# aalobaidi/ggRMCP

Hardware: AMD Instinct MI355X
Metric: MCP tool_call→gRPC unary req/sec (whole node) (higher is better)
Workload: dtype uint8; 1 GPU; model=hello-service SayHello (HTTP serving), global_batch=1024, seq_len=1024, parallelism=dp1, mode=serving-gpu, sessions=1024, payload_bytes=1024, backend=local grpc over uds, separate process (native) x1, transport=native, http=native frontend, C++ closed-loop client

## Files before the change

### ggrmcp_amd/backend/native_invoker.py

```python

from __future__ import annotations

import logging
from typing import Dict, List, Optional, Sequence, Tuple

log = logging.getLogger("ggrmcp.native_invoker")

_CODE_NAMES = [
    "OK", "CANCELLED", "UNKNOWN", "INVALID_ARGUMENT", "DEADLINE_EXCEEDED",
    "NOT_FOUND", "ALREADY_EXISTS", "PERMISSION_DENIED", "RESOURCE_EXHAUSTED",
    "FAILED_PRECONDITION", "ABORTED", "OUT_OF_RANGE", "UNIMPLEMENTED",
    "INTERNAL", "UNAVAILABLE", "DATA_LOSS", "UNAUTHENTICATED",
]


class _Code:
    def __init__(self, value: int) -> None:
        self.value = value
        self.name = (
            _CODE_NAMES[value] if 0 <= value < len(_CODE_NAMES) else f"CODE_{value}"
        )


class NativeRpcError(Exception):

    def __init__(self, code: int, message: str) -> None:
        super().__init__(f"{_Code(code).name}: {message}")
        self._code = _Code(code)
        self._message = message

    def code(self) -> _Code:
        return self._code

    def details(self) -> str:
        return self._message


def load_module():
    import importlib
    import sys
    from pathlib import Path

    ops_dir = str(Path(__file__).resolve().parent.parent / "ops")
    if ops_dir not in sys.path:
        sys.path.insert(0, ops_dir)
    return importlib.import_module("_h2grpc")


class NativeWireClient:

    def __init__(self, target: str, connections: int = 8, authority: str = "",
                 max_inflight: int = 512, max_resp_bytes: int = 0) -> None:
        mod = load_module()
        self.target = target
        self._cli = mod.Client(target, connections=connections,
                               authority=authority or "localhost",
                               max_inflight=max_inflight,
                               max_resp_bytes=max_resp_bytes)

    def invoke_batch(
        self,
        paths: Sequence[str],
        payloads: Sequence[bytes],
        timeout_s: float,
        metadata: Optional[Sequence[Sequence[Tuple[str, str]]]] = None,
    ) -> List[object]:
        res = self._cli.invoke_batch(
            list(paths), list(payloads), timeout_s, list(metadata or [])
        )
        out: List[object] = []
        for status, payload, message in res:
            if status == 0:
                out.append(payload)
            else:
                out.append(NativeRpcError(status, message))
        return out

    def invoke_stream_batch(
        self,
        paths: Sequence[str],
        payloads: Sequence[bytes],
        timeout_s: float,
        metadata: Optional[Sequence[Sequence[Tuple[str, str]]]] = None,
    ) -> List[object]:
        res = self._cli.invoke_stream_batch(
            list(paths), list(payloads), timeout_s, list(metadata or [])
        )
        out: List[object] = []
        for status, blob, lens, message in res:
            if status == 0:
                mv = memoryview(blob)
                chunks = []
                off = 0
                for ln in lens:
                    chunks.append(mv[off : off + ln])
                    off += ln
                out.append(chunks)
            else:
                out.append(NativeRpcError(status, message))
        return out

    def healthy(self) -> bool:
        return self._cli.healthy()

    def close(self) -> None:
        self._cli.close()
```

### ggrmcp_amd/ops/csrc/h2grpc.cpp

```cpp

#include "h2grpc_impl.h"

PYBIND11_MODULE(_h2grpc, m) {
  m.doc() = "native gRPC-over-HTTP/2 transport (nghttp2): batch client + bench server";
  py::class_<H2GrpcClient>(m, "Client")
      .def(py::init<const std::string&, int, const std::string&, int, size_t>(),
           py::arg("target"), py::arg("connections") = 4, py::arg("authority") = "",
           py::arg("max_inflight") = 512, py::arg("max_resp_bytes") = 0)
      .def("invoke_stream_batch", &H2GrpcClient::invoke_stream_batch,
           py::arg("paths"), py::arg("payloads"), py::arg("timeout_s") = 30.0,
           py::arg("metadata") = std::vector<std::vector<std::pair<std::string, std::string>>>{})
      .def("invoke_batch", &H2GrpcClient::invoke_batch, py::arg("paths"),
           py::arg("payloads"), py::arg("timeout_s") = 30.0,
           py::arg("metadata") = std::vector<std::vector<std::pair<std::string, std::string>>>{})
      .def("healthy", &H2GrpcClient::healthy)
      .def("raw_handle",
           [](H2GrpcClient& c) { return (uintptr_t)&c; },
           "opaque H2GrpcClient* for the native span executor; the client "
           "must outlive every frontend/engine holding the handle")
      .def("close", &H2GrpcClient::close_all);
  py::class_<H2Server>(m, "Server")
      .def(py::init<const std::string&>(), py::arg("target"))
      .def("add_route", &H2Server::add_route, py::arg("path"), py::arg("kind"))
      .def("request_count", &H2Server::request_count)
      .def("start", &H2Server::start)
      .def("stop", &H2Server::stop);
}
```

### ggrmcp_amd/ops/csrc/h2grpc_impl.h

```cpp
#pragma once

#include <arpa/inet.h>
#include <errno.h>
#include <fcntl.h>
#include <netinet/in.h>
#include <netinet/tcp.h>
#include <nghttp2/nghttp2.h>
#include <poll.h>
#include <pybind11/pybind11.h>
#include <pybind11/stl.h>
#include <string.h>
#include <stdio.h>
#include <stdlib.h>
#include <sys/eventfd.h>
#include <sys/socket.h>
#include <sys/un.h>
#include <unistd.h>

#include <atomic>
#include <chrono>
#include <condition_variable>
#include <cstdint>
#include <deque>
#include <memory>
#include <mutex>
#include <stdexcept>
#include <string>
#include <thread>
#include <unordered_map>
#include <vector>

namespace py = pybind11;
using Clock = std::chrono::steady_clock;


static int transport_sockbuf() {
  const char* e = getenv("GGRMCP_SOCKBUF");
  return e ? atoi(e) : (4 << 20);
}

static void apply_sockbuf(int fd) {
  int sz = transport_sockbuf();
  if (sz > 0) {
    setsockopt(fd, SOL_SOCKET, SO_SNDBUF, &sz, sizeof(sz));
    setsockopt(fd, SOL_SOCKET, SO_RCVBUF, &sz, sizeof(sz));
  }
}

static int connect_target(const std::string& target) {
  int fd = -1;
  if (target.rfind("unix:", 0) == 0) {
    fd = socket(AF_UNIX, SOCK_STREAM, 0);
    if (fd < 0) throw std::runtime_error("socket() failed");
    sockaddr_un addr{};
    addr.sun_family = AF_UNIX;
    std::string path = target.substr(5);
    if (path.size() >= sizeof(addr.sun_path)) throw std::runtime_error("uds path too long");
    memcpy(addr.sun_path, path.c_str(), path.size() + 1);
    apply_sockbuf(fd);
    if (connect(fd, (sockaddr*)&addr, sizeof(addr)) != 0) {
      close(fd);
      throw std::runtime_error("connect failed: " + target);
    }
  } else {
    auto colon = target.rfind(':');
    if (colon == std::string::npos) throw std::runtime_error("bad target " + target);
    std::string host = target.substr(0, colon);
    int port = std::stoi(target.substr(colon + 1));
    fd = socket(AF_INET, SOCK_STREAM, 0);
    if (fd < 0) throw std::runtime_error("socket() failed");
    sockaddr_in addr{};
    addr.sin_family = AF_INET;
    addr.sin_port = htons((uint16_t)port);
    if (inet_pton(AF_INET, host.c_str(), &addr.sin_addr) != 1) {
      close(fd);
      throw std::runtime_error("bad host (use a literal IP): " + host);
    }
    apply_sockbuf(fd);
    if (connect(fd, (sockaddr*)&addr, sizeof(addr)) != 0) {
      close(fd);
      throw std::runtime_error("connect failed: " + target);
    }
    int one = 1;
    setsockopt(fd, IPPROTO_TCP, TCP_NODELAY, &one, sizeof(one));
  }
  int flags = fcntl(fd, F_GETFL, 0);
  fcntl(fd, F_SETFL, flags | O_NONBLOCK);
  return fd;
}

#define NV(NAME, VALUE, NLEN, VLEN)                                      \
  nghttp2_nv {                                                           \
    (uint8_t*)(NAME), (uint8_t*)(VALUE), (size_t)(NLEN), (size_t)(VLEN), \
        NGHTTP2_NV_FLAG_NONE                                             \
  }

static nghttp2_nv nv(const char* name, const char* value) {
  return NV(name, value, strlen(name), strlen(value));
}
static nghttp2_nv nv(const char* name, const std::string& value) {
  return NV(name, value.data(), strlen(name), value.size());
}
static nghttp2_nv nv(const std::string& name, const std::string& value) {
  return NV(name.data(), value.data(), name.size(), value.size());
}

static std::string grpc_frame(const std::string& payload) {
  std::string out;
  out.resize(5 + payload.size());
  out[0] = 0;
  uint32_t n = htonl((uint32_t)payload.size());
  memcpy(&out[1], &n, 4);
  memcpy(&out[5], payload.data(), payload.size());
  return out;
}

static bool pb_validate(const uint8_t* p, size_t len) {
  size_t pos = 0;
  int depth_guard = 0;
  while (pos < len) {
    uint64_t tag = 0;
    int shift = 0;
    bool done = false;
    while (pos < len && shift <= 63) {
      uint8_t b = p[pos++];
      tag |= (uint64_t)(b & 0x7F) << shift;
      if (!(b & 0x80)) { done = true; break; }
      shift += 7;
    }
    if (!done) return false;
    uint32_t wt = tag & 7;
    if ((tag >> 3) == 0) return false;
    switch (wt) {
      case 0: {
        bool vdone = false;
        for (int i = 0; i < 10 && pos < len; ++i) {
          if (!(p[pos++] & 0x80)) { vdone = true; break; }
        }
        if (!vdone) return false;
        break;
      }
      case 1: if (pos + 8 > len) return false; pos += 8; break;
      case 5: if (pos + 4 > len) return false; pos += 4; break;
      case 2: {
        uint64_t l = 0;
        int s2 = 0;
        bool d2 = false;
        while (pos < len && s2 <= 35) {
          uint8_t b = p[pos++];
          l |= (uint64_t)(b & 0x7F) << s2;
          if (!(b & 0x80)) { d2 = true; break; }
          s2 += 7;
        }
        if (!d2 || pos + l > len) return false;
        pos += l;
        break;
      }
      default: return false;
    }
    if (++depth_guard > 1'000'000) return false;
  }
  return true;
}

static bool parse_hello_name(const uint8_t* p, size_t len, std::string* name) {
  size_t pos = 0;
  while (pos < len) {
    uint64_t tag = 0;
    int shift = 0;
    bool done = false;
    while (pos < len && shift <= 63) {
      uint8_t b = p[pos++];
      tag |= (uint64_t)(b & 0x7F) << shift;
      if (!(b & 0x80)) { done = true; break; }
      shift += 7;
    }
    if (!done) return false;
    if ((tag >> 3) == 1 && (tag & 7) == 2) {
      uint64_t l = 0;
      int s2 = 0;
      bool d2 = false;
      while (pos < len && s2 <= 35) {
        uint8_t b = p[pos++];
        l |= (uint64_t)(b & 0x7F) << s2;
        if (!(b & 0x80)) { d2 = true; break; }
        s2 += 7;
      }
      if (!d2 || pos + l > len) return false;
      name->assign((const char*)p + pos, l);
      pos += l;
    } else {
      uint32_t wt = tag & 7;
      if (wt == 0) {
        while (pos < len && (p[pos++] & 0x80)) {}
      } else if (wt == 1) {
        pos += 8;
      } else if (wt == 5) {
        pos += 4;
      } else if (wt == 2) {
        uint64_t l = 0;
        int s2 = 0;
        while (pos < len && s2 <= 35) {
          uint8_t b = p[pos++];
          l |= (uint64_t)(b & 0x7F) << s2;
          if (!(b & 0x80)) break;
          s2 += 7;
        }
        pos += l;
      } else {
        return false;
      }
    }
  }
  return true;
}

static std::string make_hello_response(const std::string& name) {
  std::string msg = "Hello, " + name + "!";
  std::string out;
  out.push_back('\x0a');
  uint64_t v = msg.size();
  while (v >= 0x80) {
    out.push_back((char)(v | 0x80));
    v >>= 7;
  }
  out.push_back((char)v);
  out += msg;
  return out;
}


struct Call {
  std::string path;
  std::string payload;
  size_t sent = 0;
  std::string response;
  int grpc_status = -1;
  std::string grpc_message;
  std::atomic<bool> done{false};
  Clock::time_point deadline;
  int slot = -1;
  bool no_cap = false;
  bool overflow = false;
  std::vector<std::pair<std::string, std::string>> metadata;
};

struct Batch {
  std::deque<Call> calls;
  std::mutex mu;
  std::condition_variable cv;
  std::atomic<int> done{0};
  void complete_one() {
    { std::lock_guard<std::mutex> lk(mu); done.fetch_add(1); }
    cv.notify_one();
  }
};

struct QueuedCall {
  std::shared_ptr<Batch> batch;
  Call* call;
};

struct ClientConn {
  int fd = -1;
  int wake_fd = -1;
  nghttp2_session* sess = nullptr;
  std::thread thread;
  std::mutex mu;
  std::deque<QueuedCall> pending;
  std::unordered_map<int32_t, QueuedCall> live;
  std::string wbuf;
  std::atomic<bool> stop{false};
  std::atomic<int> inflight{0};
  int max_inflight = 512;
  size_t max_resp = 0;
  std::string authority;
  bool broken = false;
};

static ssize_t client_data_read(nghttp2_session*, int32_t stream_id, uint8_t* buf,
                                size_t length, uint32_t* data_flags,
                                nghttp2_data_source* source, void*) {
  Call* call = (Call*)source->ptr;
  size_t left = call->payload.size() - call->sent;
  size_t n = left < length ? left : length;
  memcpy(buf, call->payload.data() + call->sent, n);
  call->sent += n;
  if (call->sent == call->payload.size()) *data_flags |= NGHTTP2_DATA_FLAG_EOF;
  return (ssize_t)n;
}

static int client_on_header(nghttp2_session* sess, const nghttp2_frame* frame,
                            const uint8_t* name, size_t namelen, const uint8_t* value,
                            size_t valuelen, uint8_t, void* user) {
  ClientConn* conn = (ClientConn*)user;
  auto it = conn->live.find(frame->hd.stream_id);
  if (it == conn->live.end()) return 0;
  if (namelen == 11 && memcmp(name, "grpc-status", 11) == 0) {
    it->second.call->grpc_status =
        atoi(std::string((const char*)value, valuelen).c_str());
  } else if (namelen == 12 && memcmp(name, "grpc-message", 12) == 0) {
    it->second.call->grpc_message.assign((const char*)value, valuelen);
  }
  return 0;
}

static int client_on_data(nghttp2_session*, uint8_t, int32_t stream_id,
                          const uint8_t* data, size_t len, void* user) {
  ClientConn* conn = (ClientConn*)user;
  auto it = conn->live.find(stream_id);
  if (it != conn->live.end()) {
    Call* c = it->second.call;
    if (!c->no_cap && conn->max_resp &&
        c->response.size() + len > conn->max_resp) {
      c->overflow = true;
      c->response.clear();
    } else if (!c->overflow) {
      c->response.append((const char*)data, len);
    }
  }
  return 0;
}

static int client_on_stream_close(nghttp2_session*, int32_t stream_id, uint32_t,
                                  void* user) {
  ClientConn* conn = (ClientConn*)user;
  auto it = conn->live.find(stream_id);
  if (it != conn->live.end()) {
    QueuedCall qc = it->second;
    conn->live.erase(it);
    qc.call->done.store(true, std::memory_order_release);
    conn->inflight.fetch_sub(1);
    qc.batch->complete_one();
  }
  return 0;
}

static void fail_call(ClientConn* conn, QueuedCall& qc, int status,
                      const char* msg) {
  qc.call->grpc_status = status;
  qc.call->grpc_message = msg;
  qc.call->done.store(true, std::memory_order_release);
  qc.batch->complete_one();
}


static bool flush_session(nghttp2_session* sess, int fd, std::string& wbuf,
                          bool* blocked) {
  *blocked = false;
  while (true) {
    if (!wbuf.empty()) {
      ssize_t w = send(fd, wbuf.data(), wbuf.size(), MSG_NOSIGNAL);
      if (w < 0) {
        if (errno == EAGAIN || errno == EWOULDBLOCK) { *blocked = true; return true; }
        return false;
      }
      wbuf.erase(0, (size_t)w);
      if (!wbuf.empty()) continue;
    }
    const uint8_t* out = nullptr;
    ssize_t n = nghttp2_session_mem_send(sess, &out);
    if (n < 0) return false;
    if (n == 0) return true;
    ssize_t w = send(fd, out, (size_t)n, MSG_NOSIGNAL);
    if (w < 0) {
      if (errno == EAGAIN || errno == EWOULDBLOCK) w = 0;
      else return false;
    }
    if (w < n) wbuf.assign((const char*)out + w, (size_t)(n - w));
  }
}

static void conn_loop(ClientConn* conn) {
  while (!conn->stop.load()) {
    {
      std::lock_guard<std::mutex> lk(conn->mu);
      while (!conn->pending.empty() &&
             conn->inflight.load() < conn->max_inflight) {
        QueuedCall qc = conn->pending.front();
        Call* call = qc.call;
        conn->pending.pop_front();
        std::vector<nghttp2_nv> nva;
        nva.reserve(8 + call->metadata.size());
        nva.push_back(nv(":method", "POST"));
        nva.push_back(nv(":scheme", "http"));
        nva.push_back(nv(":path", call->path));
        nva.push_back(nv(":authority", conn->authority));
        nva.push_back(nv("te", "trailers"));
        nva.push_back(nv("content-type", "application/grpc"));
        for (auto& kv : call->metadata) nva.push_back(nv(kv.first, kv.second));
        nghttp2_data_provider prd;
        prd.source.ptr = call;
        prd.read_callback = client_data_read;
        int32_t sid = nghttp2_submit_request(conn->sess, nullptr, nva.data(),
                                             nva.size(), &prd, call);
        if (sid < 0) {
          fail_call(conn, qc, 14, "submit failed");
          continue;
        }
        conn->live[sid] = qc;
        conn->inflight.fetch_add(1);
      }
    }
    {
      auto now = Clock::now();
      for (auto& kv : conn->live) {
        if (kv.second.call->deadline < now && kv.second.call->grpc_status < 0) {
          kv.second.call->grpc_status = 4;
          kv.second.call->grpc_message = "deadline exceeded";
          nghttp2_submit_rst_stream(conn->sess, NGHTTP2_FLAG_NONE, kv.first,
                                    NGHTTP2_CANCEL);
        }
      }
    }
    bool write_blocked = false;
    if (!flush_session(conn->sess, conn->fd, conn->wbuf, &write_blocked))
      conn->broken = true;
    if (conn->broken) break;

    pollfd fds[2];
    fds[0] = {conn->fd, (short)(POLLIN | (write_blocked ? POLLOUT : 0)), 0};
    fds[1] = {conn->wake_fd, POLLIN, 0};
    int rc = poll(fds, 2, 100);
    if (rc < 0) break;
    if (fds[1].revents & POLLIN) {
      uint64_t junk;
      while (read(conn->wake_fd, &junk, 8) > 0) {}
    }
    if (fds[0].revents & (POLLIN | POLLERR | POLLHUP)) {
      uint8_t buf[1 << 16];
      while (true) {
        ssize_t r = recv(conn->fd, buf, sizeof(buf), 0);
        if (r > 0) {
          ssize_t consumed = nghttp2_session_mem_recv(conn->sess, buf, r);
          if (consumed < 0) { conn->broken = true; break; }
          if (r < (ssize_t)sizeof(buf)) break;
        } else if (r == 0) {
          conn->broken = true;
          break;
        } else {
          if (errno == EAGAIN || errno == EWOULDBLOCK) break;
          conn->broken = true;
          break;
        }
      }
    }
    if (conn->broken) break;
  }
  std::lock_guard<std::mutex> lk(conn->mu);
  for (auto& kv : conn->live) fail_call(conn, kv.second, 14, "connection lost");
  for (auto& qc : conn->pending) fail_call(conn, qc, 14, "connection lost");
  conn->live.clear();
  conn->pending.clear();
}

class __attribute__((visibility("default"))) H2GrpcClient {
 public:
  H2GrpcClient(const std::string& target, int n_connections,
               const std::string& authority, int max_inflight = 512,
               size_t max_resp_bytes = 0)
      : target_(target) {
    if (n_connections < 1) n_connections = 1;
    for (int i = 0; i < n_connections; ++i) {
      auto conn = std::make_unique<ClientConn>();
      conn->max_inflight = max_inflight < 1 ? 1 : max_inflight;
      conn->max_resp = max_resp_bytes;
      conn->fd = connect_target(target);
      conn->wake_fd = eventfd(0, EFD_NONBLOCK);
      conn->authority = authority.empty() ? "localhost" : authority;

      nghttp2_session_callbacks* cbs;
      nghttp2_session_callbacks_new(&cbs);
      nghttp2_session_callbacks_set_on_header_callback(cbs, client_on_header);
      nghttp2_session_callbacks_set_on_data_chunk_recv_callback(cbs, client_on_data);
      nghttp2_session_callbacks_set_on_stream_close_callback(cbs, client_on_stream_close);
      nghttp2_session_client_new(&conn->sess, cbs, conn.get());
      nghttp2_session_callbacks_del(cbs);

      nghttp2_settings_entry iv[] = {
          {NGHTTP2_SETTINGS_INITIAL_WINDOW_SIZE, (1u << 30)},
          {NGHTTP2_SETTINGS_MAX_CONCURRENT_STREAMS, 8192},
          {NGHTTP2_SETTINGS_MAX_FRAME_SIZE, 1u << 20},
      };
      nghttp2_submit_settings(conn->sess, NGHTTP2_FLAG_NONE, iv, 3);
      nghttp2_session_set_local_window_size(conn->sess, NGHTTP2_FLAG_NONE, 0, 1 << 30);

      ClientConn* raw = conn.get();
      conn->thread = std::thread([raw] { conn_loop(raw); });
      conns_.push_back(std::move(conn));
    }
  }

  ~H2GrpcClient() { close_all(); }

  void close_all() {
    for (auto& conn : conns_) {
      conn->stop.store(true);
      uint64_t one = 1;
      (void)!write(conn->wake_fd, &one, 8);
      if (conn->thread.joinable()) conn->thread.join();
      if (conn->sess) nghttp2_session_del(conn->sess);
      if (conn->fd >= 0) close(conn->fd);
      if (conn->wake_fd >= 0) close(conn->wake_fd);
      conn->sess = nullptr;
      conn->fd = conn->wake_fd = -1;
    }
    conns_.clear();
  }

  bool healthy() const {
    for (auto& conn : conns_)
      if (!conn->broken) return true;
    return false;
  }

// ... 15 lines not shown
      size_t pos = 0;
      bool compressed = false;
      while (pos + 5 <= data.size()) {
        if (data[pos] != 0) {
          compressed = true;
          break;
        }
        uint32_t len;
        memcpy(&len, data.data() + pos + 1, 4);
        len = ntohl(len);
        if (pos + 5 + len > data.size()) break;
        blob.append(data, pos + 5, len);
        lens.push_back(len);
        pos += 5 + len;
      }
      if (status == 0 && compressed) {
        status = 13;
        std::get<2>(r) = "compressed gRPC response frame not supported";
      }
      if (status < 0) {
        status = 2;
        if (std::get<2>(r).empty())
          std::get<2>(r) = "stream closed without grpc-status";
      }
      out.emplace_back(status, py::bytes(blob), std::move(lens), std::get<2>(r));
    }
    return out;
  }

  std::vector<std::tuple<int, py::bytes, std::string>> invoke_batch(
      const std::vector<std::string>& paths, const std::vector<py::bytes>& payloads,
      double timeout_s,
      const std::vector<std::vector<std::pair<std::string, std::string>>>& metadata) {
    auto raw = invoke_collect(paths, payloads, timeout_s, metadata);
    std::vector<std::tuple<int, py::bytes, std::string>> out;
    out.reserve(raw.size());
    for (auto& r : raw) {
      int status = std::get<0>(r);
      const std::string& data = std::get<1>(r);
      std::string payload;
      bool compressed = false;
      if (data.size() >= 5) {
        compressed = data[0] != 0;
        uint32_t len;
        memcpy(&len, data.data() + 1, 4);
        len = ntohl(len);
        if (data.size() >= 5 + (size_t)len) payload = data.substr(5, len);
      }
      if (status < 0) {
        status = 2;
        if (std::get<2>(r).empty())
          std::get<2>(r) = "stream closed without grpc-status";
      } else if (status == 0 && compressed) {
        status = 13;
        std::get<2>(r) = "compressed gRPC response frame not supported";
        payload.clear();
      }
      out.emplace_back(status, py::bytes(payload), std::get<2>(r));
    }
    return out;
  }

 public:
  struct RawCall {
    const char* path;
    size_t path_len;
    const uint8_t* payload;
    size_t payload_len;
    const std::vector<std::pair<std::string, std::string>>* metadata;
  };
  std::vector<std::tuple<int, std::string, std::string>> invoke_raw(
      const std::vector<RawCall>& rc, double timeout_s) {
    size_t n = rc.size();
    auto batch = std::make_shared<Batch>();
    auto deadline = Clock::now() + std::chrono::duration_cast<Clock::duration>(
                                       std::chrono::duration<double>(timeout_s));
    for (size_t i = 0; i < n; ++i) {
      batch->calls.emplace_back();
      Call& call = batch->calls.back();
      call.path.assign(rc[i].path, rc[i].path_len);
      call.deadline = deadline;
      call.slot = (int)i;
      if (rc[i].metadata) call.metadata = *rc[i].metadata;
      call.payload = grpc_frame(
          std::string((const char*)rc[i].payload, rc[i].payload_len));
    }
    size_t nc = conns_.size();
    for (size_t i = 0; i < n; ++i) {
      ClientConn* conn = conns_[i % nc].get();
      std::lock_guard<std::mutex> lk(conn->mu);
      conn->pending.push_back(QueuedCall{batch, &batch->calls[i]});
    }
    for (auto& conn : conns_) {
      uint64_t one = 1;
      (void)!write(conn->wake_fd, &one, 8);
    }
    {
      std::unique_lock<std::mutex> lk(batch->mu);
      auto hard = deadline + std::chrono::seconds(2);
      while (batch->done.load() < (int)n) {
        if (batch->cv.wait_until(lk, hard) == std::cv_status::timeout) break;
      }
    }
    std::vector<std::tuple<int, std::string, std::string>> out;
    out.reserve(n);
    for (size_t i = 0; i < n; ++i) {
      Call& call = batch->calls[i];
      if (!call.done.load(std::memory_order_acquire)) {
        out.emplace_back(4, std::string(), "deadline exceeded");
        continue;
      }
      if (call.overflow) {
        out.emplace_back(8, std::string(),
                         "response exceeds max_recv_msg_bytes");
        continue;
      }
      out.emplace_back(call.grpc_status, std::move(call.response),
                       call.grpc_message);
    }
    return out;
  }

 private:
  std::vector<std::tuple<int, std::string, std::string>> invoke_collect(
      const std::vector<std::string>& paths, const std::vector<py::bytes>& payloads,
      double timeout_s,
      const std::vector<std::vector<std::pair<std::string, std::string>>>& metadata,
      bool no_cap = false) {
    size_t n = paths.size();
    if (payloads.size() != n) throw std::runtime_error("paths/payloads mismatch");
    auto batch = std::make_shared<Batch>();
    auto deadline = Clock::now() + std::chrono::duration_cast<Clock::duration>(
                                       std::chrono::duration<double>(timeout_s));
    for (size_t i = 0; i < n; ++i) {
      batch->calls.emplace_back();
      Call& call = batch->calls.back();
      call.path = paths[i];
      call.deadline = deadline;
      call.slot = (int)i;
      call.no_cap = no_cap;
      if (i < metadata.size()) call.metadata = metadata[i];
      std::string raw = payloads[i];
      call.payload = grpc_frame(raw);
    }
    {
      py::gil_scoped_release rel;
      size_t nc = conns_.size();
      for (size_t i = 0; i < n; ++i) {
        ClientConn* conn = conns_[i % nc].get();
        std::lock_guard<std::mutex> lk(conn->mu);
        conn->pending.push_back(QueuedCall{batch, &batch->calls[i]});
      }
      for (auto& conn : conns_) {
        uint64_t one = 1;
        (void)!write(conn->wake_fd, &one, 8);
      }
      std::unique_lock<std::mutex> lk(batch->mu);
      auto hard = deadline + std::chrono::seconds(2);
      while (batch->done.load() < (int)n) {
        if (batch->cv.wait_until(lk, hard) == std::cv_status::timeout) break;
      }
    }
    std::vector<std::tuple<int, std::string, std::string>> out;
    out.reserve(n);
    for (size_t i = 0; i < n; ++i) {
      Call& call = batch->calls[i];
      if (!call.done.load(std::memory_order_acquire)) {
        out.emplace_back(4, std::string(), "deadline exceeded");
        continue;
      }
      if (call.overflow) {
        out.emplace_back(8, std::string(),
                         "response exceeds max_recv_msg_bytes");
        continue;
      }
      out.emplace_back(call.grpc_status, std::move(call.response),
                       call.grpc_message);
    }
    return out;
  }

 public:

 private:
  std::string target_;
  std::vector<std::unique_ptr<ClientConn>> conns_;
};


struct ServerStream {
  std::string path;
  std::string body;
  std::string response;
  size_t sent = 0;
  int grpc_status = 0;
  std::string grpc_message;
  bool responded = false;
};

struct ServerConn {
  int fd = -1;
  nghttp2_session* sess = nullptr;
  std::unordered_map<int32_t, ServerStream> streams;
  std::string wbuf;
  bool broken = false;
  class H2Server* server = nullptr;
};

class H2Server {
 public:
  std::unordered_map<std::string, int> routes;

  H2Server(const std::string& target) : target_(target) {}

  ~H2Server() { stop(); }

  void add_route(const std::string& path, const std::string& kind) {
    routes[path] = (kind == "hello") ? 1 : (kind == "stream_echo") ? 2 : 0;
  }

  std::string start() {
    if (target_.rfind("unix:", 0) == 0) {
      listen_fd_ = socket(AF_UNIX, SOCK_STREAM, 0);
      sockaddr_un addr{};
      addr.sun_family = AF_UNIX;
      std::string path = target_.substr(5);
      if (path.size() >= sizeof(addr.sun_path))
        throw std::runtime_error("uds path too long: " + path);
      unlink(path.c_str());
      memcpy(addr.sun_path, path.c_str(), path.size() + 1);
      if (bind(listen_fd_, (sockaddr*)&addr, sizeof(addr)) != 0)
        throw std::runtime_error("bind failed: " + target_);
      bound_ = target_;
    } else {
      auto colon = target_.rfind(':');
      std::string host = target_.substr(0, colon);
      int port = std::stoi(target_.substr(colon + 1));
      listen_fd_ = socket(AF_INET, SOCK_STREAM, 0);
      int one = 1;
      setsockopt(listen_fd_, SOL_SOCKET, SO_REUSEADDR, &one, sizeof(one));
      sockaddr_in addr{};
      addr.sin_family = AF_INET;
      addr.sin_port = htons((uint16_t)port);
      inet_pton(AF_INET, host.c_str(), &addr.sin_addr);
      if (bind(listen_fd_, (sockaddr*)&addr, sizeof(addr)) != 0)
        throw std::runtime_error("bind failed: " + target_);
      socklen_t alen = sizeof(addr);
      getsockname(listen_fd_, (sockaddr*)&addr, &alen);
      bound_ = host + ":" + std::to_string(ntohs(addr.sin_port));
    }
    if (listen(listen_fd_, 512) != 0) throw std::runtime_error("listen failed");
    int flags = fcntl(listen_fd_, F_GETFL, 0);
    fcntl(listen_fd_, F_SETFL, flags | O_NONBLOCK);
    stop_.store(false);
    accept_thread_ = std::thread([this] { accept_loop(); });
    return bound_;
  }

  void stop() {
    if (stop_.exchange(true)) return;
    if (accept_thread_.joinable()) accept_thread_.join();
    if (listen_fd_ >= 0) close(listen_fd_);
    listen_fd_ = -1;
  }

  long request_count() const { return requests_.load(); }

  void handle(ServerStream& st) {
    requests_.fetch_add(1, std::memory_order_relaxed);
    auto it = routes.find(st.path);
    if (it == routes.end()) {
      st.grpc_status = 12;
      st.grpc_message = "unknown method " + st.path;
      return;
    }
    if (st.body.size() < 5) {
      st.grpc_status = 13;
      st.grpc_message = "truncated grpc frame";
      return;
    }
    uint32_t len;
    memcpy(&len, st.body.data() + 1, 4);
    len = ntohl(len);
    if (st.body.size() < 5 + (size_t)len) {
      st.grpc_status = 13;
      st.grpc_message = "short grpc frame";
      return;
    }
    const uint8_t* msg = (const uint8_t*)st.body.data() + 5;
    if (it->second == 2) {
      if (!pb_validate(msg, len)) {
        st.grpc_status = 13;
        st.grpc_message = "malformed protobuf";
        return;
      }
      int64_t count = 1;
      {
        size_t pos = 0;
        while (pos < len) {
          uint64_t tag = 0;
          int shift = 0;
          while (pos < len && shift <= 63) {
            uint8_t b = msg[pos++];
            tag |= (uint64_t)(b & 0x7F) << shift;
            if (!(b & 0x80)) break;
            shift += 7;
          }
          uint32_t num = (uint32_t)(tag >> 3), wt = (uint32_t)(tag & 7);
          if (num == 2 && wt == 0) {
            uint64_t v = 0;
            int s2 = 0;
            while (pos < len && s2 <= 63) {
              uint8_t b = msg[pos++];
              v |= (uint64_t)(b & 0x7F) << s2;
              if (!(b & 0x80)) break;
              s2 += 7;
            }
            count = (int64_t)(int32_t)(uint32_t)v;
            break;
          }
          if (wt == 0) {
            while (pos < len && (msg[pos++] & 0x80)) {}
          } else if (wt == 1) {
            pos += 8;
          } else if (wt == 5) {
            pos += 4;
          } else if (wt == 2) {
            uint64_t l = 0;
            int s2 = 0;
            while (pos < len && s2 <= 35) {
              uint8_t b = msg[pos++];
              l |= (uint64_t)(b & 0x7F) << s2;
              if (!(b & 0x80)) break;
              s2 += 7;
            }
            pos += l;
          } else {
            break;
          }
        }
      }
      if (count < 1) count = 1;
      if (count > 65536) count = 65536;
      std::string one = grpc_frame(std::string((const char*)msg, len));
      st.response.reserve(one.size() * count);
      for (int64_t i = 0; i < count; ++i) st.response += one;
      return;
    }
    if (it->second == 1) {
      std::string name;
      if (!parse_hello_name(msg, len, &name)) {
        st.grpc_status = 13;
        st.grpc_message = "bad HelloRequest";
        return;
      }
      if (name == "error") {
        st.grpc_status = 3;
        st.grpc_message = "name must not be 'error'";
        return;
      }
      if (name == "badutf8") {
        std::string msg = "bad\xff\xfe";
        std::string out;
        out.push_back('\x0a');
        out.push_back((char)msg.size());
        out += msg;
        st.response = grpc_frame(out);
        return;
      }
      st.response = grpc_frame(make_hello_response(name));
    } else {
      if (!pb_validate(msg, len)) {
        st.grpc_status = 13;
        st.grpc_message = "malformed protobuf";
        return;
      }
      st.response = grpc_frame(std::string((const char*)msg, len));
    }
  }

 private:
  void accept_loop() {
    std::vector<std::thread> workers;
    while (!stop_.load()) {
      pollfd pfd{listen_fd_, POLLIN, 0};
      int rc = poll(&pfd, 1, 200);
      if (rc <= 0) continue;
      int cfd = accept(listen_fd_, nullptr, nullptr);
      if (cfd < 0) continue;
      int flags = fcntl(cfd, F_GETFL, 0);
      fcntl(cfd, F_SETFL, flags | O_NONBLOCK);
      int one = 1;
      setsockopt(cfd, IPPROTO_TCP, TCP_NODELAY, &one, sizeof(one));
      apply_sockbuf(cfd);
      workers.emplace_back([this, cfd] { conn_loop(cfd); });
    }
    for (auto& t : workers)
      if (t.joinable()) t.join();
  }

  static ssize_t resp_read(nghttp2_session* sess, int32_t stream_id, uint8_t* buf,
                           size_t length, uint32_t* data_flags,
                           nghttp2_data_source* source, void*) {
    ServerStream* st = (ServerStream*)source->ptr;
    size_t left = st->response.size() - st->sent;
    size_t n = left < length ? left : length;
    memcpy(buf, st->response.data() + st->sent, n);
    st->sent += n;
    if (st->sent == st->response.size()) {
      *data_flags |= NGHTTP2_DATA_FLAG_EOF | NGHTTP2_DATA_FLAG_NO_END_STREAM;
      std::string status = std::to_string(st->grpc_status);
      std::vector<nghttp2_nv> trailers;
      trailers.push_back(nv("grpc-status", status));
      if (!st->grpc_message.empty())
        trailers.push_back(nv("grpc-message", st->grpc_message));
      nghttp2_submit_trailer(sess, stream_id, trailers.data(), trailers.size());
    }
    return (ssize_t)n;
  }

  void respond(ServerConn* conn, int32_t sid, ServerStream& st) {
    handle(st);
    std::string status = std::to_string(st.grpc_status);
    if (st.grpc_status != 0 || st.response.empty()) {
      std::vector<nghttp2_nv> hdrs;
      hdrs.push_back(nv(":status", "200"));
      hdrs.push_back(nv("content-type", "application/grpc"));
      hdrs.push_back(nv("grpc-status", status));
      if (!st.grpc_message.empty())
        hdrs.push_back(nv("grpc-message", st.grpc_message));
      nghttp2_submit_response(conn->sess, sid, hdrs.data(), hdrs.size(), nullptr);
      return;
    }
    nghttp2_nv hdrs[] = {nv(":status", "200"), nv("content-type", "application/grpc")};
    nghttp2_data_provider prd;
    prd.source.ptr = &st;
    prd.read_callback = resp_read;
    nghttp2_submit_response(conn->sess, sid, hdrs, 2, &prd);
  }

  static int s_on_begin_headers(nghttp2_session*, const nghttp2_frame* frame, void* user) {
    ServerConn* conn = (ServerConn*)user;
    if (frame->hd.type == NGHTTP2_HEADERS &&
        frame->headers.cat == NGHTTP2_HCAT_REQUEST)
      conn->streams[frame->hd.stream_id];
    return 0;
  }

  static int s_on_header(nghttp2_session*, const nghttp2_frame* frame,
                         const uint8_t* name, size_t namelen, const uint8_t* value,
                         size_t valuelen, uint8_t, void* user) {
    ServerConn* conn = (ServerConn*)user;
    auto it = conn->streams.find(frame->hd.stream_id);
    if (it == conn->streams.end()) return 0;
    if (namelen == 5 && memcmp(name, ":path", 5) == 0)
      it->second.path.assign((const char*)value, valuelen);
    return 0;
  }

  static int s_on_data(nghttp2_session*, uint8_t, int32_t stream_id,
                       const uint8_t* data, size_t len, void* user) {
    ServerConn* conn = (ServerConn*)user;
    auto it = conn->streams.find(stream_id);
    if (it != conn->streams.end()) it->second.body.append((const char*)data, len);
    return 0;
  }

  static int s_on_frame_recv(nghttp2_session*, const nghttp2_frame* frame, void* user) {
    ServerConn* conn = (ServerConn*)user;
    if ((frame->hd.type == NGHTTP2_DATA || frame->hd.type == NGHTTP2_HEADERS) &&
        (frame->hd.flags & NGHTTP2_FLAG_END_STREAM)) {
      auto it = conn->streams.find(frame->hd.stream_id);
      if (it != conn->streams.end() && !it->second.responded) {
        it->second.responded = true;
        conn->server->respond(conn, frame->hd.stream_id, it->second);
      }
    }
    return 0;
  }

  static int s_on_stream_close(nghttp2_session*, int32_t stream_id, uint32_t,
                               void* user) {
    ServerConn* conn = (ServerConn*)user;
    conn->streams.erase(stream_id);
    return 0;
  }

  void conn_loop(int cfd) {
    ServerConn conn;
    conn.fd = cfd;
    conn.server = this;
    nghttp2_session_callbacks* cbs;
    nghttp2_session_callbacks_new(&cbs);
    nghttp2_session_callbacks_set_on_begin_headers_callback(cbs, s_on_begin_headers);
    nghttp2_session_callbacks_set_on_header_callback(cbs, s_on_header);
    nghttp2_session_callbacks_set_on_data_chunk_recv_callback(cbs, s_on_data);
    nghttp2_session_callbacks_set_on_frame_recv_callback(cbs, s_on_frame_recv);
    nghttp2_session_callbacks_set_on_stream_close_callback(cbs, s_on_stream_close);
    nghttp2_session_server_new(&conn.sess, cbs, &conn);
    nghttp2_session_callbacks_del(cbs);
    nghttp2_settings_entry iv[] = {
        {NGHTTP2_SETTINGS_INITIAL_WINDOW_SIZE, (1u << 30)},
        {NGHTTP2_SETTINGS_MAX_CONCURRENT_STREAMS, 8192},
        {NGHTTP2_SETTINGS_MAX_FRAME_SIZE, 1u << 20},
    };
    nghttp2_submit_settings(conn.sess, NGHTTP2_FLAG_NONE, iv, 3);
    nghttp2_session_set_local_window_size(conn.sess, NGHTTP2_FLAG_NONE, 0, 1 << 30);

    while (!stop_.load() && !conn.broken) {
      bool write_blocked = false;
      if (!flush_session(conn.sess, conn.fd, conn.wbuf, &write_blocked))
        conn.broken = true;
      if (conn.broken) break;
      pollfd pfd{conn.fd, (short)(POLLIN | (write_blocked ? POLLOUT : 0)), 0};
      int rc = poll(&pfd, 1, 200);
      if (rc < 0) break;
      if (pfd.revents & (POLLIN | POLLERR | POLLHUP)) {
        uint8_t buf[1 << 16];
        while (true) {
          ssize_t r = recv(conn.fd, buf, sizeof(buf), 0);
          if (r > 0) {
            if (nghttp2_session_mem_recv(conn.sess, buf, r) < 0) {
              conn.broken = true;
              break;
            }
            if (r < (ssize_t)sizeof(buf)) break;
          } else if (r == 0) {
            conn.broken = true;
            break;
          } else {
            if (errno == EAGAIN || errno == EWOULDBLOCK) break;
            conn.broken = true;
            break;
          }
        }
      }
      if (nghttp2_session_want_read(conn.sess) == 0 &&
          nghttp2_session_want_write(conn.sess) == 0)
        break;
    }
    nghttp2_session_del(conn.sess);
    close(cfd);
  }

  std::string target_;
  std::string bound_;
  int listen_fd_ = -1;
  std::thread accept_thread_;
  std::atomic<bool> stop_{true};
  std::atomic<long> requests_{0};
};
```

Measured before the change: 399,500 req/s.

## Batch nghttp2 writes with gather buffer and cut per-call transport overheads

```diff
diff --git a/ggrmcp_amd/backend/native_invoker.py b/ggrmcp_amd/backend/native_invoker.py
--- a/ggrmcp_amd/backend/native_invoker.py
+++ b/ggrmcp_amd/backend/native_invoker.py
@@ -103,5 +103,8 @@
     def healthy(self) -> bool:
         return self._cli.healthy()
 
+    def stats(self) -> Dict[str, int]:
+        return dict(self._cli.stats())
+
     def close(self) -> None:
         self._cli.close()
diff --git a/ggrmcp_amd/ops/csrc/h2grpc.cpp b/ggrmcp_amd/ops/csrc/h2grpc.cpp
--- a/ggrmcp_amd/ops/csrc/h2grpc.cpp
+++ b/ggrmcp_amd/ops/csrc/h2grpc.cpp
@@ -3,6 +3,8 @@
 
 PYBIND11_MODULE(_h2grpc, m) {
   m.doc() = "native gRPC-over-HTTP/2 transport (nghttp2): batch client + bench server";
+  m.attr("GATHER_CAP") = (size_t)kGatherCap;
+  m.attr("DIRECT_SEND_MIN") = (size_t)kDirectSendMin;
   py::class_<H2GrpcClient>(m, "Client")
       .def(py::init<const std::string&, int, const std::string&, int, size_t>(),
            py::arg("target"), py::arg("connections") = 4, py::arg("authority") = "",
@@ -14,6 +16,9 @@
            py::arg("payloads"), py::arg("timeout_s") = 30.0,
            py::arg("metadata") = std::vector<std::vector<std::pair<std::string, std::string>>>{})
       .def("healthy", &H2GrpcClient::healthy)
+      .def("stats", &H2GrpcClient::stats,
+           "transport counters: calls, batches, send_calls, send_bytes, "
+           "recv_calls, wake_writes, notifies")
       .def("raw_handle",
            [](H2GrpcClient& c) { return (uintptr_t)&c; },
            "opaque H2GrpcClient* for the native span executor; the client "
@@ -23,6 +28,8 @@
       .def(py::init<const std::string&>(), py::arg("target"))
       .def("add_route", &H2Server::add_route, py::arg("path"), py::arg("kind"))
       .def("request_count", &H2Server::request_count)
+      .def("stats", &H2Server::stats,
+           "transport counters: calls, send_calls, send_bytes, recv_calls")
       .def("start", &H2Server::start)
       .def("stop", &H2Server::stop);
 }
diff --git a/ggrmcp_amd/ops/csrc/h2grpc_impl.h b/ggrmcp_amd/ops/csrc/h2grpc_impl.h
--- a/ggrmcp_amd/ops/csrc/h2grpc_impl.h
+++ b/ggrmcp_amd/ops/csrc/h2grpc_impl.h
@@ -14,6 +14,7 @@
 #include <stdlib.h>
 #include <sys/eventfd.h>
 #include <sys/socket.h>
+#include <sys/uio.h>
 #include <sys/un.h>
 #include <unistd.h>
 
@@ -105,15 +106,71 @@
   return NV(name.data(), value.data(), name.size(), value.size());
 }
 
+static void grpc_frame_into(std::string& out, const void* payload, size_t len) {
+  out.resize(5 + len);
+  out[0] = 0;
+  uint32_t n = htonl((uint32_t)len);
+  memcpy(&out[1], &n, 4);
+  if (len) memcpy(&out[5], payload, len);
+}
 static std::string grpc_frame(const std::string& payload) {
   std::string out;
-  out.resize(5 + payload.size());
-  out[0] = 0;
-  uint32_t n = htonl((uint32_t)payload.size());
-  memcpy(&out[1], &n, 4);
-  memcpy(&out[5], payload.data(), payload.size());
+  grpc_frame_into(out, payload.data(), payload.size());
   return out;
 }
+
+#define GGRMCP_H2_STATS 1
+struct TransportStats {
+  std::atomic<uint64_t> calls{0};
+  std::atomic<uint64_t> batches{0};
+  std::atomic<uint64_t> send_calls{0};
+  std::atomic<uint64_t> send_bytes{0};
+  std::atomic<uint64_t> recv_calls{0};
+  std::atomic<uint64_t> wake_writes{0};
+  std::atomic<uint64_t> notifies{0};
+  static void bump(std::atomic<uint64_t>& c, uint64_t v = 1) {
+    c.fetch_add(v, std::memory_order_relaxed);
+  }
+  void add_into(std::unordered_map<std::string, uint64_t>& m) const {
+    auto ld = [](const std::atomic<uint64_t>& c) {
+      return c.load(std::memory_order_relaxed);
+    };
+    m["calls"] += ld(calls);
+    m["batches"] += ld(batches);
+    m["send_calls"] += ld(send_calls);
+    m["send_bytes"] += ld(send_bytes);
+    m["recv_calls"] += ld(recv_calls);
+    m["wake_writes"] += ld(wake_writes);
+    m["notifies"] += ld(notifies);
+  }
+};
+
+#ifndef H2_GATHER_CAP
+#define H2_GATHER_CAP (256u << 10)
+#endif
+#ifndef H2_DIRECT_SEND_MIN
+#define H2_DIRECT_SEND_MIN (8u << 10)
+#endif
+static constexpr size_t kGatherCap = H2_GATHER_CAP;
+static constexpr size_t kDirectSendMin = H2_DIRECT_SEND_MIN;
+static constexpr int kBulkHoldPasses = 8;
+
+static constexpr int kDefaultConnRun = 1;
+static int transport_conn_run() {
+  static const int v = [] {
+    const char* e = getenv("GGRMCP_H2_RUN");
+    int k = e ? atoi(e) : kDefaultConnRun;
+    return k < 1 ? 1 : k;
+  }();
+  return v;
+}
+
+struct WriteBuf {
+  std::string buf;
+  size_t off = 0;
+  int bulk = 0;
+  size_t pending() const { return buf.size() - off; }
+};
 
 static bool pb_validate(const uint8_t* p, size_t len) {
   size_t pos = 0;
@@ -215,18 +272,26 @@
   return true;
 }
 
-static std::string make_hello_response(const std::string& name) {
-  std::string msg = "Hello, " + name + "!";
-  std::string out;
-  out.push_back('\x0a');
-  uint64_t v = msg.size();
-  while (v >= 0x80) {
-    out.push_back((char)(v | 0x80));
-    v >>= 7;
-  }
-  out.push_back((char)v);
-  out += msg;
-  return out;
+static void hello_response_into(std::string& out, const std::string& name) {
+  size_t mlen = 7 + name.size() + 1;
+  char var[10];
+  size_t nvar = 0;
+  for (uint64_t v = mlen;; v >>= 7) {
+    if (v >= 0x80) { var[nvar++] = (char)(v | 0x80); }
+    else { var[nvar++] = (char)v; break; }
+  }
+  size_t pblen = 1 + nvar + mlen;
+  out.resize(5 + pblen);
+  char* p = &out[0];
+  *p++ = 0;
+  uint32_t be = htonl((uint32_t)pblen);
+  memcpy(p, &be, 4); p += 4;
+  *p++ = '\x0a';
+  memcpy(p, var, nvar); p += nvar;
+  memcpy(p, "Hello, ", 7); p += 7;
+  if (!name.empty()) memcpy(p, name.data(), name.size());
+  p += name.size();
+  *p = '!';
 }
 
 
@@ -250,9 +315,18 @@
   std::mutex mu;
   std::condition_variable cv;
   std::atomic<int> done{0};
+  int total = 0;
+  TransportStats* stats = nullptr;
   void complete_one() {
-    { std::lock_guard<std::mutex> lk(mu); done.fetch_add(1); }
-    cv.notify_one();
+    bool last;
+    {
+      std::lock_guard<std::mutex> lk(mu);
+      last = done.fetch_add(1) + 1 >= total;
+    }
+    if (last) {
+      if (stats) TransportStats::bump(stats->notifies);
+      cv.notify_one();
+    }
   }
 };
 
@@ -269,8 +343,10 @@
   std::mutex mu;
   std::deque<QueuedCall> pending;
   std::unordered_map<int32_t, QueuedCall> live;
-  std::string wbuf;
+  WriteBuf wbuf;
+  TransportStats stats;
   std::atomic<bool> stop{false};
+  std::atomic<bool> sleeping{false};
   std::atomic<int> inflight{0};
   int max_inflight = 512;
   size_t max_resp = 0;
@@ -290,27 +366,37 @@
   return (ssize_t)n;
 }
 
+static int parse_status(const uint8_t* v, size_t n) {
+  size_t i = 0;
+  while (i < n && (v[i] == ' ' || (v[i] >= '\t' && v[i] <= '\r'))) ++i;
+  bool neg = false;
+  if (i < n && (v[i] == '-' || v[i] == '+')) neg = v[i++] == '-';
+  int r = 0;
+  for (; i < n && v[i] >= '0' && v[i] <= '9' && r < 100000000; ++i)
+    r = r * 10 + (v[i] - '0');
+  return neg ? -r : r;
+}
+
 static int client_on_header(nghttp2_session* sess, const nghttp2_frame* frame,
                             const uint8_t* name, size_t namelen, const uint8_t* value,
                             size_t valuelen, uint8_t, void* user) {
-  ClientConn* conn = (ClientConn*)user;
-  auto it = conn->live.find(frame->hd.stream_id);
-  if (it == conn->live.end()) return 0;
+  (void)user;
+  Call* call =
+      (Call*)nghttp2_session_get_stream_user_data(sess, frame->hd.stream_id);
+  if (!call) return 0;
   if (namelen == 11 && memcmp(name, "grpc-status", 11) == 0) {
-    it->second.call->grpc_status =
-        atoi(std::string((const char*)value, valuelen).c_str());
+    call->grpc_status = parse_status(value, valuelen);
   } else if (namelen == 12 && memcmp(name, "grpc-message", 12) == 0) {
-    it->second.call->grpc_message.assign((const char*)value, valuelen);
+    call->grpc_message.assign((const char*)value, valuelen);
   }
   return 0;
 }
 
-static int client_on_data(nghttp2_session*, uint8_t, int32_t stream_id,
+static int client_on_data(nghttp2_session* sess, uint8_t, int32_t stream_id,
                           const uint8_t* data, size_t len, void* user) {
   ClientConn* conn = (ClientConn*)user;
-  auto it = conn->live.find(stream_id);
-  if (it != conn->live.end()) {
-    Call* c = it->second.call;
+  Call* c = (Call*)nghttp2_session_get_stream_user_data(sess, stream_id);
+  if (c) {
     if (!c->no_cap && conn->max_resp &&
         c->response.size() + len > conn->max_resp) {
       c->overflow = true;
@@ -327,7 +413,7 @@
   ClientConn* conn = (ClientConn*)user;
   auto it = conn->live.find(stream_id);
   if (it != conn->live.end()) {
-    QueuedCall qc = it->second;
+    QueuedCall qc = std::move(it->second);
     conn->live.erase(it);
     qc.call->done.store(true, std::memory_order_release);
     conn->inflight.fetch_sub(1);
@@ -345,29 +431,75 @@
 }
 
 
-static bool flush_session(nghttp2_session* sess, int fd, std::string& wbuf,
-                          bool* blocked) {
+static int wb_send(int fd, WriteBuf& wb, const uint8_t* extra, size_t xn,
+                   TransportStats* st) {
+  while (true) {
+    size_t pend = wb.pending();
+    if (pend == 0) {
+      wb.buf.clear();
+      wb.off = 0;
+      if (xn == 0) return 1;
+    }
+    ssize_t w;
+    if (xn == 0) {
+      w = send(fd, wb.buf.data() + wb.off, pend, MSG_NOSIGNAL);
+    } else if (pend == 0) {
+      w = send(fd, extra, xn, MSG_NOSIGNAL);
+    } else {
+      iovec iov[2] = {{(void*)(wb.buf.data() + wb.off), pend},
+                      {(void*)extra, xn}};
+      msghdr mh{};
+      mh.msg_iov = iov;
+      mh.msg_iovlen = 2;
+      w = sendmsg(fd, &mh, MSG_NOSIGNAL);
+    }
+    TransportStats::bump(st->send_calls);
+    if (w < 0) {
+      if (errno == EINTR) continue;
+      if (errno == EAGAIN || errno == EWOULDBLOCK) {
+        if (xn) wb.buf.append((const char*)extra, xn);
+        return 0;
+      }
+      return -1;
+    }
+    TransportStats::bump(st->send_bytes, (uint64_t)w);
+    size_t from_buf = (size_t)w < pend ? (size_t)w : pend;
+    wb.off += from_buf;
+    extra += (size_t)w - from_buf;
+    xn -= (size_t)w - from_buf;
+  }
+}
+
+static bool flush_session(nghttp2_session* sess, int fd, WriteBuf& wb,
+                          bool* blocked, TransportStats* st) {
   *blocked = false;
+  bool sent_any = false, saw_big = false;
   while (true) {
-    if (!wbuf.empty()) {
-      ssize_t w = send(fd, wbuf.data(), wbuf.size(), MSG_NOSIGNAL);
-      if (w < 0) {
-        if (errno == EAGAIN || errno == EWOULDBLOCK) { *blocked = true; return true; }
-        return false;
-      }
-      wbuf.erase(0, (size_t)w);
-      if (!wbuf.empty()) continue;
-    }
-    const uint8_t* out = nullptr;
-    ssize_t n = nghttp2_session_mem_send(sess, &out);
-    if (n < 0) return false;
-    if (n == 0) return true;
-    ssize_t w = send(fd, out, (size_t)n, MSG_NOSIGNAL);
-    if (w < 0) {
-      if (errno == EAGAIN || errno == EWOULDBLOCK) w = 0;
-      else return false;
-    }
-    if (w < n) wbuf.assign((const char*)out + w, (size_t)(n - w));
+    int r = wb_send(fd, wb, nullptr, 0, st);
+    if (r < 0) return false;
+    if (r == 0) { *blocked = true; return true; }
+    while (wb.buf.size() < kGatherCap) {
+      const uint8_t* out = nullptr;
+      ssize_t n = nghttp2_session_mem_send(sess, &out);
+      if (n < 0) return false;
+      if (n == 0) {
+        if (!wb.buf.empty()) break;
+        if (sent_any && !saw_big && wb.bulk > 0) --wb.bulk;
+        return true;
+      }
+      sent_any = true;
+      if ((size_t)n >= kDirectSendMin) {
+        saw_big = true;
+        wb.bulk = kBulkHoldPasses;
+      }
+      if (wb.bulk > 0) {
+        r = wb_send(fd, wb, out, (size_t)n, st);
+        if (r < 0) return false;
+        if (r == 0) { *blocked = true; return true; }
+        continue;
+      }
+      wb.buf.append((const char*)out, (size_t)n);
+    }
   }
 }
 
@@ -377,28 +509,36 @@
       std::lock_guard<std::mutex> lk(conn->mu);
       while (!conn->pending.empty() &&
              conn->inflight.load() < conn->max_inflight) {
-        QueuedCall qc = conn->pending.front();
+        QueuedCall qc = std::move(conn->pending.front());
         Call* call = qc.call;
         conn->pending.pop_front();
-        std::vector<nghttp2_nv> nva;
-        nva.reserve(8 + call->metadata.size());
-        nva.push_back(nv(":method", "POST"));
-        nva.push_back(nv(":scheme", "http"));
-        nva.push_back(nv(":path", call->path));
-        nva.push_back(nv(":authority", conn->authority));
-        nva.push_back(nv("te", "trailers"));
-        nva.push_back(nv("content-type", "application/grpc"));
-        for (auto& kv : call->metadata) nva.push_back(nv(kv.first, kv.second));
+        nghttp2_nv fixed[6] = {
+            NV(":method", "POST", 7, 4),
+            NV(":scheme", "http", 7, 4),
+            nv(":path", call->path),
+            nv(":authority", conn->authority),
+            NV("te", "trailers", 2, 8),
+            NV("content-type", "application/grpc", 12, 16),
+        };
+        const nghttp2_nv* nva = fixed;
+        size_t nvlen = 6;
+        std::vector<nghttp2_nv> with_md;
+        if (!call->metadata.empty()) {
+          with_md.assign(fixed, fixed + 6);
+          for (auto& kv : call->metadata) with_md.push_back(nv(kv.first, kv.second));
+          nva = with_md.data();
+          nvlen = with_md.size();
+        }
         nghttp2_data_provider prd;
         prd.source.ptr = call;
         prd.read_callback = client_data_read;
-        int32_t sid = nghttp2_submit_request(conn->sess, nullptr, nva.data(),
-                                             nva.size(), &prd, call);
+        int32_t sid = nghttp2_submit_request(conn->sess, nullptr, nva, nvlen,
+                                             &prd, call);
         if (sid < 0) {
           fail_call(conn, qc, 14, "submit failed");
           continue;
         }
-        conn->live[sid] = qc;
+        conn->live[sid] = std::move(qc);
         conn->inflight.fetch_add(1);
       }
     }
@@ -414,15 +554,29 @@
       }
     }
     bool write_blocked = false;
-    if (!flush_session(conn->sess, conn->fd, conn->wbuf, &write_blocked))
+    if (!flush_session(conn->sess, conn->fd, conn->wbuf, &write_blocked,
+                       &conn->stats))
       conn->broken = true;
     if (conn->broken) break;
 
+    conn->sleeping.store(true, std::memory_order_seq_cst);
+    {
+      std::lock_guard<std::mutex> lk(conn->mu);
+      if (!conn->pending.empty() &&
+          conn->inflight.load() < conn->max_inflight) {
+        conn->sleeping.store(false, std::memory_order_relaxed);
+        continue;
+      }
+    }
     pollfd fds[2];
     fds[0] = {conn->fd, (short)(POLLIN | (write_blocked ? POLLOUT : 0)), 0};
     fds[1] = {conn->wake_fd, POLLIN, 0};
     int rc = poll(fds, 2, 100);
-    if (rc < 0) break;
+    conn->sleeping.store(false, std::memory_order_seq_cst);
+    if (rc < 0) {
+      if (errno == EINTR) continue;
+      break;
+    }
     if (fds[1].revents & POLLIN) {
       uint64_t junk;
       while (read(conn->wake_fd, &junk, 8) > 0) {}
@@ -431,6 +585,7 @@
       uint8_t buf[1 << 16];
       while (true) {
         ssize_t r = recv(conn->fd, buf, sizeof(buf), 0);
+        TransportStats::bump(conn->stats.recv_calls);
         if (r > 0) {
           ssize_t consumed = nghttp2_session_mem_recv(conn->sess, buf, r);
           if (consumed < 0) { conn->broken = true; break; }
@@ -612,30 +767,61 @@
       call.deadline = deadline;
       call.slot = (int)i;
       if (rc[i].metadata) call.metadata = *rc[i].metadata;
-      call.payload = grpc_frame(
-          std::string((const char*)rc[i].payload, rc[i].payload_len));
-    }
+      grpc_frame_into(call.payload, rc[i].payload, rc[i].payload_len);
+    }
+    submit_and_wait(batch, n, deadline);
+    return collect(*batch, n);
+  }
+
+  std::unordered_map<std::string, uint64_t> stats() const {
+    std::unordered_map<std::string, uint64_t> m;
+    stats_.add_into(m);
+    for (auto& conn : conns_) conn->stats.add_into(m);
+    return m;
+  }
+
+ private:
+  void submit_and_wait(const std::shared_ptr<Batch>& batch, size_t n,
+                       Clock::time_point deadline) {
+    batch->total = (int)n;
+    batch->stats = &stats_;
+    TransportStats::bump(stats_.batches);
+    TransportStats::bump(stats_.calls, n);
     size_t nc = conns_.size();
-    for (size_t i = 0; i < n; ++i) {
-      ClientConn* conn = conns_[i % nc].get();
-      std::lock_guard<std::mutex> lk(conn->mu);
-      conn->pending.push_back(QueuedCall{batch, &batch->calls[i]});
-    }
-    for (auto& conn : conns_) {
-      uint64_t one = 1;
-      (void)!write(conn->wake_fd, &one, 8);
-    }
-    {
-      std::unique_lock<std::mutex> lk(batch->mu);
-      auto hard = deadline + std::chrono::seconds(2);
-      while (batch->done.load() < (int)n) {
-        if (batch->cv.wait_until(lk, hard) == std::cv_status::timeout) break;
-      }
-    }
+    if (nc == 0 && n) throw std::runtime_error("client is closed");
+    size_t run = (size_t)transport_conn_run();
+    size_t start = next_conn_.fetch_add(1, std::memory_order_relaxed);
+    size_t nruns = (n + run - 1) / run;
+    size_t used = nruns < nc ? nruns : nc;
+    for (size_t j = 0; j < used; ++j) {
+      ClientConn* conn = conns_[(start + j) % nc].get();
+      {
+        std::lock_guard<std::mutex> lk(conn->mu);
+        for (size_t r = j; r < nruns; r += nc) {
+          size_t end = (r + 1) * run < n ? (r + 1) * run : n;
+          for (size_t i = r * run; i < end; ++i)
+            conn->pending.push_back(QueuedCall{batch, &batch->calls[i]});
+        }
+      }
+      if (conn->sleeping.load(std::memory_order_seq_cst)) {
+        uint64_t one = 1;
+        (void)!write(conn->wake_fd, &one, 8);
+        TransportStats::bump(stats_.wake_writes);
+      }
+    }
+    std::unique_lock<std::mutex> lk(batch->mu);
+    auto hard = deadline + std::chrono::seconds(2);
+    while (batch->done.load() < (int)n) {
+      if (batch->cv.wait_until(lk, hard) == std::cv_status::timeout) break;
+    }
+  }
+
+  static std::vector<std::tuple<int, std::string, std::string>> collect(
+      Batch& batch, size_t n) {
     std::vector<std::tuple<int, std::string, std::string>> out;
     out.reserve(n);
     for (size_t i = 0; i < n; ++i) {
-      Call& call = batch->calls[i];
+      Call& call = batch.calls[i];
       if (!call.done.load(std::memory_order_acquire)) {
         out.emplace_back(4, std::string(), "deadline exceeded");
         continue;
@@ -651,7 +837,6 @@
     return out;
   }
 
- private:
   std::vector<std::tuple<int, std::string, std::string>> invoke_collect(
       const std::vector<std::string>& paths, const std::vector<py::bytes>& payloads,
       double timeout_s,
@@ -670,51 +855,23 @@
       call.slot = (int)i;
       call.no_cap = no_cap;
       if (i < metadata.size()) call.metadata = metadata[i];
-      std::string raw = payloads[i];
-      call.payload = grpc_frame(raw);
+      char* data = nullptr;
+      Py_ssize_t len = 0;
+      if (PyBytes_AsStringAndSize(payloads[i].ptr(), &data, &len) != 0)
+        throw py::error_already_set();
+      grpc_frame_into(call.payload, data, (size_t)len);
     }
     {
       py::gil_scoped_release rel;
-      size_t nc = conns_.size();
-      for (size_t i = 0; i < n; ++i) {
-        ClientConn* conn = conns_[i % nc].get();
-        std::lock_guard<std::mutex> lk(conn->mu);
-        conn->pending.push_back(QueuedCall{batch, &batch->calls[i]});
-      }
-      for (auto& conn : conns_) {
-        uint64_t one = 1;
-        (void)!write(conn->wake_fd, &one, 8);
-      }
-      std::unique_lock<std::mutex> lk(batch->mu);
-      auto hard = deadline + std::chrono::seconds(2);
-      while (batch->done.load() < (int)n) {
-        if (batch->cv.wait_until(lk, hard) == std::cv_status::timeout) break;
-      }
-    }
-    std::vector<std::tuple<int, std::string, std::string>> out;
-    out.reserve(n);
-    for (size_t i = 0; i < n; ++i) {
-      Call& call = batch->calls[i];
-      if (!call.done.load(std::memory_order_acquire)) {
-        out.emplace_back(4, std::string(), "deadline exceeded");
-        continue;
-      }
-      if (call.overflow) {
-        out.emplace_back(8, std::string(),
-                         "response exceeds max_recv_msg_bytes");
-        continue;
-      }
-      out.emplace_back(call.grpc_status, std::move(call.response),
-                       call.grpc_message);
-    }
-    return out;
-  }
-
- public:
-
- private:
+      submit_and_wait(batch, n, deadline);
+    }
+    return collect(*batch, n);
+  }
+
   std::string target_;
   std::vector<std::unique_ptr<ClientConn>> conns_;
+  TransportStats stats_;
+  std::atomic<size_t> next_conn_{0};
 };
 
 
@@ -732,7 +889,7 @@
   int fd = -1;
   nghttp2_session* sess = nullptr;
   std::unordered_map<int32_t, ServerStream> streams;
-  std::string wbuf;
+  WriteBuf wbuf;
   bool broken = false;
   class H2Server* server = nullptr;
 };
@@ -795,6 +952,13 @@
   }
 
   long request_count() const { return requests_.load(); }
+
+  std::unordered_map<std::string, uint64_t> stats() const {
+    std::unordered_map<std::string, uint64_t> m;
+    stats_.add_into(m);
+    m["calls"] = (uint64_t)requests_.load(std::memory_order_relaxed);
+    return m;
+  }
 
   void handle(ServerStream& st) {
     requests_.fetch_add(1, std::memory_order_relaxed);
@@ -872,7 +1036,8 @@
       }
       if (count < 1) count = 1;
       if (count > 65536) count = 65536;
-      std::string one = grpc_frame(std::string((const char*)msg, len));
+      std::string one;
+      grpc_frame_into(one, msg, len);
       st.response.reserve(one.size() * count);
       for (int64_t i = 0; i < count; ++i) st.response += one;
       return;
@@ -898,14 +1063,14 @@
         st.response = grpc_frame(out);
         return;
       }
-      st.response = grpc_frame(make_hello_response(name));
+      hello_response_into(st.response, name);
     } else {
       if (!pb_validate(msg, len)) {
         st.grpc_status = 13;
         st.grpc_message = "malformed protobuf";
         return;
       }
-      st.response = grpc_frame(std::string((const char*)msg, len));
+      grpc_frame_into(st.response, msg, len);
     }
   }
 
@@ -939,79 +1104,85 @@
     st->sent += n;
     if (st->sent == st->response.size()) {
       *data_flags |= NGHTTP2_DATA_FLAG_EOF | NGHTTP2_DATA_FLAG_NO_END_STREAM;
-      std::string status = std::to_string(st->grpc_status);
-      std::vector<nghttp2_nv> trailers;
-      trailers.push_back(nv("grpc-status", status));
+      nghttp2_nv trailers[2] = {NV("grpc-status", "0", 11, 1), {}};
+      size_t nt = 1;
       if (!st->grpc_message.empty())
-        trailers.push_back(nv("grpc-message", st->grpc_message));
-      nghttp2_submit_trailer(sess, stream_id, trailers.data(), trailers.size());
+        trailers[nt++] = nv("grpc-message", st->grpc_message);
+      nghttp2_submit_trailer(sess, stream_id, trailers, nt);
     }
     return (ssize_t)n;
   }
 
   void respond(ServerConn* conn, int32_t sid, ServerStream& st) {
     handle(st);
-    std::string status = std::to_string(st.grpc_status);
     if (st.grpc_status != 0 || st.response.empty()) {
-      std::vector<nghttp2_nv> hdrs;
-      hdrs.push_back(nv(":status", "200"));
-      hdrs.push_back(nv("content-type", "application/grpc"));
-      hdrs.push_back(nv("grpc-status", status));
+      char status[16];
+      int slen = snprintf(status, sizeof(status), "%d", st.grpc_status);
+      nghttp2_nv hdrs[4] = {
+          NV(":status", "200", 7, 3),
+          NV("content-type", "application/grpc", 12, 16),
+          NV("grpc-status", status, 11, slen),
+          {},
+      };
+      size_t nh = 3;
       if (!st.grpc_message.empty())
-        hdrs.push_back(nv("grpc-message", st.grpc_message));
-      nghttp2_submit_response(conn->sess, sid, hdrs.data(), hdrs.size(), nullptr);
+        hdrs[nh++] = nv("grpc-message", st.grpc_message);
+      nghttp2_submit_response(conn->sess, sid, hdrs, nh, nullptr);
       return;
     }
-    nghttp2_nv hdrs[] = {nv(":status", "200"), nv("content-type", "application/grpc")};
+    nghttp2_nv hdrs[] = {NV(":status", "200", 7, 3),
+                         NV("content-type", "application/grpc", 12, 16)};
     nghttp2_data_provider prd;
     prd.source.ptr = &st;
     prd.read_callback = resp_read;
     nghttp2_submit_response(conn->sess, sid, hdrs, 2, &prd);
   }
 
-  static int s_on_begin_headers(nghttp2_session*, const nghttp2_frame* frame, void* user) {
+  static int s_on_begin_headers(nghttp2_session* sess, const nghttp2_frame* frame, void* user) {
     ServerConn* conn = (ServerConn*)user;
     if (frame->hd.type == NGHTTP2_HEADERS &&
         frame->headers.cat == NGHTTP2_HCAT_REQUEST)
-      conn->streams[frame->hd.stream_id];
+      nghttp2_session_set_stream_user_data(sess, frame->hd.stream_id,
+                                           &conn->streams[frame->hd.stream_id]);
     return 0;
   }
 
-  static int s_on_header(nghttp2_session*, const nghttp2_frame* frame,
+  static int s_on_header(nghttp2_session* sess, const nghttp2_frame* frame,
                          const uint8_t* name, size_t namelen, const uint8_t* value,
-                         size_t valuelen, uint8_t, void* user) {
-    ServerConn* conn = (ServerConn*)user;
-    auto it = conn->streams.find(frame->hd.stream_id);
-    if (it == conn->streams.end()) return 0;
-    if (namelen == 5 && memcmp(name, ":path", 5) == 0)
-      it->second.path.assign((const char*)value, valuelen);
+                         size_t valuelen, uint8_t, void*) {
+    ServerStream* st = (ServerStream*)nghttp2_session_get_stream_user_data(
+        sess, frame->hd.stream_id);
+    if (st && namelen == 5 && memcmp(name, ":path", 5) == 0)
+      st->path.assign((const char*)value, valuelen);
     return 0;
   }
 
-  static int s_on_data(nghttp2_session*, uint8_t, int32_t stream_id,
-                       const uint8_t* data, size_t len, void* user) {
-    ServerConn* conn = (ServerConn*)user;
-    auto it = conn->streams.find(stream_id);
-    if (it != conn->streams.end()) it->second.body.append((const char*)data, len);
+  static int s_on_data(nghttp2_session* sess, uint8_t, int32_t stream_id,
+                       const uint8_t* data, size_t len, void*) {
+    ServerStream* st =
+        (ServerStream*)nghttp2_session_get_stream_user_data(sess, stream_id);
+    if (st) st->body.append((const char*)data, len);
     return 0;
   }
 
-  static int s_on_frame_recv(nghttp2_session*, const nghttp2_frame* frame, void* user) {
+  static int s_on_frame_recv(nghttp2_session* sess, const nghttp2_frame* frame, void* user) {
     ServerConn* conn = (ServerConn*)user;
     if ((frame->hd.type == NGHTTP2_DATA || frame->hd.type == NGHTTP2_HEADERS) &&
         (frame->hd.flags & NGHTTP2_FLAG_END_STREAM)) {
-      auto it = conn->streams.find(frame->hd.stream_id);
-      if (it != conn->streams.end() && !it->second.responded) {
-        it->second.responded = true;
-        conn->server->respond(conn, frame->hd.stream_id, it->second);
+      ServerStream* st = (ServerStream*)nghttp2_session_get_stream_user_data(
+          sess, frame->hd.stream_id);
+      if (st && !st->responded) {
+        st->responded = true;
+        conn->server->respond(conn, frame->hd.stream_id, *st);
       }
     }
     return 0;
   }
 
-  static int s_on_stream_close(nghttp2_session*, int32_t stream_id, uint32_t,
+  static int s_on_stream_close(nghttp2_session* sess, int32_t stream_id, uint32_t,
                                void* user) {
     ServerConn* conn = (ServerConn*)user;
+    nghttp2_session_set_stream_user_data(sess, stream_id, nullptr);
     conn->streams.erase(stream_id);
     return 0;
   }
@@ -1039,7 +1210,7 @@
 
     while (!stop_.load() && !conn.broken) {
       bool write_blocked = false;
-      if (!flush_session(conn.sess, conn.fd, conn.wbuf, &write_blocked))
+      if (!flush_session(conn.sess, conn.fd, conn.wbuf, &write_blocked, &stats_))
         conn.broken = true;
       if (conn.broken) break;
       pollfd pfd{conn.fd, (short)(POLLIN | (write_blocked ? POLLOUT : 0)), 0};
@@ -1049,6 +1220,7 @@
         uint8_t buf[1 << 16];
         while (true) {
           ssize_t r = recv(conn.fd, buf, sizeof(buf), 0);
+          TransportStats::bump(stats_.recv_calls);
           if (r > 0) {
             if (nghttp2_session_mem_recv(conn.sess, buf, r) < 0) {
               conn.broken = true;
@@ -1079,4 +1251,5 @@
   std::thread accept_thread_;
   std::atomic<bool> stop_{true};
   std::atomic<long> requests_{0};
+  TransportStats stats_;
 };
```

After: 451,600 req/s (median of 6 runs). +13.0%, better.
